# tgm-team/tgm

Hardware: AMD Instinct MI355X
Metric: sampled-edges/sec (TGAT 2-hop k=20 recency sampler, tgbl-wiki synthetic) (higher is better)
Workload: dtype int32/int64 indices + f32 feature rows (copied, no arithmetic)

## Files before the change

### include/tgm_amd.h

```cpp
#ifndef TGM_AMD_H
#define TGM_AMD_H

#include <stddef.h>
#include <stdint.h>

#ifdef __cplusplus
extern "C" {
#endif

#define TGMX_ABI_VERSION 7

#define TGMX_OK 0
#define TGMX_E_INVALID (-1)
#define TGMX_E_LAUNCH (-2)
#define TGMX_E_UNSUPPORTED (-3)

#define TGMX_ST_SEED_RANGE 1
#define TGMX_ST_SEED_TIME 2
#define TGMX_ST_EDGE_RANGE 4
#define TGMX_ST_SCRATCH 8
#define TGMX_ST_TS_BOUND 16

typedef void* tgmx_stream_t;
typedef void* tgmx_event_t;
// ... 69 lines not shown
  float* out_x[TGMX_MAX_HOPS];
  const int32_t* src;
  const int32_t* dst;
  const int64_t* ts;
  const float* edge_x;
  int64_t n, eid0;
  int32_t directed, key_wrap32;
  int32_t* scratch;
  int32_t* status;
  int32_t timed_hop;
  tgmx_event_t ev_start, ev_stop;
  int64_t ts_bound;
  int32_t neg_group, neg_low, neg_high;
  uint64_t neg_seed, neg_call;
  int32_t* neg_out;
  int64_t* neg_time_out;
  int32_t guard_seed_errors;
  int32_t sorted_ts;
  int32_t* out_valid[TGMX_MAX_HOPS];
  int32_t* out_valid_prev[TGMX_MAX_HOPS];
  int64_t neg_index0;
  int64_t* csr_cursor;
  int32_t csr_x_by_pos;
  int32_t* out_eid[TGMX_MAX_HOPS];
  struct tgmx_defer* defer;
  int32_t defer_ok;
} tgmx_recency_step_t;

int tgmx_recency_step(const tgmx_recency_step_t* step, tgmx_stream_t stream);
#define TGMX_PLAN_FUSED01 1
#define TGMX_RIDE_NONE 0
#define TGMX_RIDE_SORT 1
#define TGMX_RIDE_MERGE 2
#define TGMX_RIDE_SORT_MERGE 3
#define TGMX_RIDE_PLACE_ONLY 4
#define TGMX_RIDE_ALL 5
#define TGMX_RIDE_SORT_MERGE_PLACE 6
#define TGMX_RIDE_MERGE_PLACE 7
#define TGMX_AFTER_NONE 0
#define TGMX_AFTER_COMMIT 1
#define TGMX_AFTER_PRESORTED 2
#define TGMX_AFTER_MERGE_PRESORTED 3
#define TGMX_AFTER_BLOCK 4
#define TGMX_AFTER_LARGE 5
int tgmx_recency_step_plan(const tgmx_recency_step_t* step);

typedef struct tgmx_defer tgmx_defer_t;
tgmx_defer_t* tgmx_defer_create(int32_t num_nodes, int32_t B);
void tgmx_defer_destroy(tgmx_defer_t* d);
int tgmx_defer_pending(const tgmx_defer_t* d);
int64_t tgmx_defer_count(const tgmx_defer_t* d);
int tgmx_defer_flush(tgmx_defer_t* d, tgmx_stream_t stream);
int32_t tgmx_set_fused_rows(int32_t rows);

#define TGMX_SEED_SRC 0
#define TGMX_SEED_DST 1
#define TGMX_SEED_NEG 2
typedef struct tgmx_pipeline {
  const int32_t* src;
  const int32_t* dst;
  const int64_t* ts;
  const float* edge_x;
  int64_t num_edges;
  int32_t rank, world;
  int32_t n_roles;
  int32_t seed_role[TGMX_MAX_SEED_GROUPS];
  int32_t neg_low, neg_high;
  uint64_t neg_seed;
  int32_t update;
  int32_t reserved0;
  tgmx_recency_step_t step;
} tgmx_pipeline_t;

typedef struct tgmx_pipeline_out {
  int32_t* neg;
  int64_t* neg_time;
  int32_t* seed_nid0;
  int64_t* seed_ts0;
  int32_t* out_nid[TGMX_MAX_HOPS];
  int64_t* out_ts[TGMX_MAX_HOPS];
  float* out_x[TGMX_MAX_HOPS];
  int32_t timed_hop;
  tgmx_event_t ev_start, ev_stop;
  int32_t* out_valid[TGMX_MAX_HOPS];
  int32_t* out_valid_prev[TGMX_MAX_HOPS];
  int32_t* out_eid[TGMX_MAX_HOPS];
} tgmx_pipeline_out_t;

typedef struct tgmx_pipeline_post {
  int32_t dedup;
  int32_t dedup_neg, dedup_nbr;
  int32_t num_nodes;
  void* dedup_ws;
  int32_t* uniq_out;
  int32_t edge_hop;
  int64_t edge_cap;
  int64_t* row_off;
  int64_t* edge_index;
  int64_t* edge_t;
  float* edge_x;
  int64_t* dev_sizes;
  int64_t* host_sizes;
  tgmx_event_t sizes_ready;
} tgmx_pipeline_post_t;

typedef void* tgmx_worker_t;
// ... 778 lines not shown
```

### tgm_amd/_native.py

```python
from __future__ import annotations

import ctypes
import os
from ctypes import c_char_p, c_int32, c_int64, c_size_t, c_void_p
from typing import Optional

import torch

from .exceptions import NativeLibraryError

_HERE = os.path.dirname(os.path.abspath(__file__))
LIB_PATH = os.path.join(_HERE, 'csrc', 'libtgm_amd.so')

_P = c_void_p
SIGNATURES = {
    'tgmx_version': (c_int32, []),
    'tgmx_abi_sizeof': (c_size_t, [c_int32]),
    'tgmx_last_error': (c_char_p, []),
    'tgmx_event_create': (c_int32, [ctypes.POINTER(c_void_p)]),
    'tgmx_event_destroy': (c_int32, [_P]),
    'tgmx_event_elapsed_ms': (c_int32, [_P, _P, ctypes.POINTER(ctypes.c_float)]),
    'tgmx_recency_lookup_csr': (
        c_int32,
        [_P, _P, _P, c_int32, _P, _P, c_int64, c_int32, c_int32, c_int64, c_int64, c_int32, c_int32, _P, _P, _P, _P, _P, _P, _P],
# ... 243 lines not shown
        ('table', c_void_p), ('ch', c_void_p * 4), ('ldch', c_int64 * 4),
        ('x', c_void_p), ('y', c_void_p), ('x1', c_void_p), ('att', c_void_p), ('qkv', c_void_p), ('h', c_void_p), ('mean', c_void_p),
        ('ldx', c_int64), ('ldq', c_int64), ('ldh', c_int64),
        ('out', c_void_p),
    ]


class TconvFwd(ctypes.Structure):

    _fields_ = [
        ('x', c_void_p), ('U', c_int64), ('in_ch', c_int32), ('last_update_local', c_void_p),
        ('src', c_void_p), ('tgt', c_void_p), ('t', c_void_p), ('msg', c_void_p), ('E', c_int64), ('D', c_int32), ('T', c_int32),
        ('tw', c_void_p), ('tb', c_void_p), ('W4', c_void_p), ('b4', c_void_p), ('W_edge', c_void_p), ('H', c_int32), ('C', c_int32),
        ('edge_attr', c_void_p), ('qkvs', c_void_p), ('eproj', c_void_p), ('order', c_void_p), ('seg_lo', c_void_p), ('seg_hi', c_void_p),
        ('sort_ws', c_void_p), ('sort_ws_bytes', c_size_t), ('status', c_void_p),
        ('tgt_count', c_void_p), ('cursor', c_void_p), ('order_big', c_void_p),
    ]


SEED_SRC, SEED_DST, SEED_NEG = 0, 1, 2


class Pipeline(ctypes.Structure):

    _fields_ = [
        ('src', c_void_p), ('dst', c_void_p), ('ts', c_void_p), ('edge_x', c_void_p), ('num_edges', c_int64),
        ('rank', c_int32), ('world', c_int32), ('n_roles', c_int32), ('seed_role', c_int32 * MAX_SEED_GROUPS),
        ('neg_low', c_int32), ('neg_high', c_int32), ('neg_seed', ctypes.c_uint64),
        ('update', c_int32), ('reserved0', c_int32), ('step', RecencyStep),
    ]


class PipelineOut(ctypes.Structure):

    _fields_ = [
        ('neg', c_void_p), ('neg_time', c_void_p), ('seed_nid0', c_void_p), ('seed_ts0', c_void_p),
        ('out_nid', c_void_p * MAX_HOPS), ('out_ts', c_void_p * MAX_HOPS), ('out_x', c_void_p * MAX_HOPS),
        ('timed_hop', c_int32), ('ev_start', c_void_p), ('ev_stop', c_void_p),
        ('out_valid', c_void_p * MAX_HOPS), ('out_valid_prev', c_void_p * MAX_HOPS), ('out_eid', c_void_p * MAX_HOPS),
    ]


ACCOUNTING_PARTIALS = 1024
SIGNATURES['tgmx_lookup_accounting'] = (c_int32, [_P, c_int64, _P, _P, c_int64, _P, _P])
SIGNATURES['tgmx_uniform_lookup_csr'] = (c_int32, [_P, _P, _P, c_int32, _P, c_int64, c_int32, c_int64, c_int32, c_int32, ctypes.c_uint64, ctypes.c_uint64,
                                                   _P, _P, _P, _P, _P])
SIGNATURES['tgmx_ring_update_scratch_bytes'] = (c_size_t, [c_int64, c_int32])
SIGNATURES['tgmx_defer_create'] = (c_void_p, [c_int32, c_int32])
SIGNATURES['tgmx_defer_destroy'] = (None, [_P])
SIGNATURES['tgmx_defer_pending'] = (c_int32, [_P])
SIGNATURES['tgmx_defer_count'] = (c_int64, [_P])
SIGNATURES['tgmx_defer_flush'] = (c_int32, [_P, _P])
SIGNATURES['tgmx_set_fused_rows'] = (c_int32, [c_int32])
SIGNATURES['tgmx_tgn_gru_gate_backward'] = (c_int32, [_P, _P, _P, _P, c_int32, c_int64, _P, _P, _P])
SIGNATURES['tgmx_tgn_aggregate_backward'] = (c_int32, [c_int64, _P, _P, _P, _P, _P, _P, c_int32, c_int32, _P, _P, c_int32, c_int32, _P, _P, _P])
SIGNATURES['tgmx_tconv_edge_attr_backward'] = (c_int32, [_P, _P, _P, _P, _P, _P, c_int32, c_int32, c_int64, _P, _P])
SIGNATURES['tgmx_tconv_attend_backward'] = (c_int32, [_P, _P, _P, _P, _P, _P, _P, _P, c_int64, c_int32, c_int32, ctypes.c_float, _P, _P, _P, _P, _P, _P, _P])
SIGNATURES['tgmx_group_ids'] = (c_int32, [_P, c_int32, _P, _P, _P, _P, _P, _P])
SIGNATURES['tgmx_group_ids_workspace_bytes'] = (c_size_t, [c_int64])
SIGNATURES['tgmx_group_ids_large'] = (c_int32, [_P, c_int64, _P, _P, _P, _P, _P, _P, c_size_t, _P])
SIGNATURES['tgmx_random_negatives'] = (c_int32, [c_int32, c_int32, c_int64, ctypes.c_uint64, ctypes.c_uint64, _P, _P, c_int64, _P, _P])
SIGNATURES['tgmx_random_negatives_at'] = (c_int32, [c_int32, c_int32, c_int64, ctypes.c_uint64, ctypes.c_uint64, c_int64, _P, _P, c_int64, _P, _P])
SIGNATURES['tgmx_unique_ids_workspace_bytes'] = (c_size_t, [c_int32])
SIGNATURES['tgmx_unique_ids'] = (c_int32, [_P, _P, c_int32, c_int32, _P, _P, _P, _P, _P])
SIGNATURES['tgmx_csr_build_workspace_bytes'] = (c_size_t, [c_int64, c_int32, c_int32])
SIGNATURES['tgmx_csr_build'] = (c_int32, [_P, _P, _P, c_int64, c_int32, _P, c_int64, c_int32, _P, _P, _P, c_size_t, _P, _P])
SIGNATURES['tgmx_recency_step'] = (c_int32, [ctypes.POINTER(RecencyStep), _P])
SIGNATURES['tgmx_recency_step_plan'] = (c_int32, [ctypes.POINTER(RecencyStep)])
SIGNATURES['tgmx_pipeline_step'] = (c_int32, [ctypes.POINTER(Pipeline), c_int64, c_int64, ctypes.c_uint64, ctypes.POINTER(PipelineOut), ctypes.POINTER(PipelinePost), _P])
SIGNATURES['tgmx_event_synchronize'] = (c_int32, [_P])
SIGNATURES['tgmx_event_create_sync'] = (c_int32, [ctypes.POINTER(c_void_p)])
SIGNATURES['tgmx_event_record'] = (c_int32, [_P, _P])
SIGNATURES['tgmx_stream_wait_event'] = (c_int32, [_P, _P])
SIGNATURES['tgmx_stream_handoff'] = (c_int32, [_P, _P, _P])
SIGNATURES['tgmx_worker_create'] = (c_int32, [ctypes.POINTER(c_void_p)])
SIGNATURES['tgmx_worker_destroy'] = (c_int32, [_P])
SIGNATURES['tgmx_worker_pipeline_step'] = (c_int32, [_P, ctypes.POINTER(Pipeline), c_int64, c_int64, ctypes.c_uint64, ctypes.POINTER(PipelineOut),
                                                     ctypes.POINTER(PipelinePost), _P, _P, _P, ctypes.POINTER(ctypes.c_uint64)])
SIGNATURES['tgmx_worker_wait'] = (c_int32, [_P, ctypes.c_uint64])
SIGNATURES['tgmx_slice'] = (c_int32, [_P, c_int64, c_int32, c_int64, c_int32, c_int64, c_int64, c_int64, ctypes.POINTER(c_int64), ctypes.POINTER(c_int64)])
SIGNATURES['tgmx_discretize_workspace_bytes'] = (c_size_t, [c_int64])
SIGNATURES['tgmx_discretize_keep'] = (c_int32, [_P, _P, _P, c_int64, ctypes.c_double, _P, _P, _P, _P, c_size_t, _P])
SIGNATURES['tgmx_tgn_memory_forward'] = (c_int32, [ctypes.POINTER(TgnMemoryFwd), _P])
SIGNATURES['tgmx_tconv_forward'] = (c_int32, [ctypes.POINTER(TconvFwd), _P])
SIGNATURES['tgmx_tgn_step'] = (c_int32, [ctypes.POINTER(TgnStep), _P])
SIGNATURES['tgmx_segment_sort_workspace_bytes'] = (c_size_t, [c_int64])
SIGNATURES['tgmx_segment_sort'] = (c_int32, [_P, c_int64, c_int32, _P, _P, _P, _P, c_size_t, _P, _P])
SIGNATURES['tgmx_tgat_tile16_floats'] = (c_size_t, [c_int32, c_int32])
SIGNATURES['tgmx_tgat_tile16'] = (c_int32, [_P, c_int64, c_int32, c_int32, _P, _P])
SIGNATURES['tgmx_pack2d'] = (c_int32, [ctypes.POINTER(PackJob), c_int32, _P])

SIGNATURES['tgmx_pair_dedup_workspace_bytes'] = (c_size_t, [c_int64])
SIGNATURES['tgmx_pair_dedup'] = (c_int32, [_P, _P, c_int64, _P, _P, _P, _P, _P, c_size_t, _P])
SIGNATURES['tgmx_tgat_layout'] = (c_int32, [ctypes.POINTER(TgatModel), c_int64, ctypes.POINTER(TgatHop), c_int32, ctypes.POINTER(TgatLayout)])
SIGNATURES['tgmx_tgat_workspace_bytes'] = (c_size_t, [ctypes.POINTER(TgatModel), c_int64, ctypes.POINTER(TgatHop)])
SIGNATURES['tgmx_tgat_backward_workspace_bytes'] = (c_size_t, [ctypes.POINTER(TgatModel), ctypes.POINTER(TgatLayout), ctypes.POINTER(TgatHop)])
SIGNATURES['tgmx_tgat_backward'] = (c_int32, [ctypes.POINTER(TgatModel), ctypes.POINTER(TgatLayout), ctypes.POINTER(TgatHop), _P, _P, c_int64,
                                              ctypes.POINTER(Dropout), ctypes.POINTER(TgatGrads), _P, c_size_t, _P])
SIGNATURES['tgmx_tgat_forward'] = (
    c_int32,
    [ctypes.POINTER(TgatModel), _P, c_int64, _P, c_int64, ctypes.POINTER(TgatHop), _P, c_size_t, c_int32, _P, _P],
)

SIGNATURES['tgmx_sgemm_nt_ep'] = (c_int32, [_P, c_int64, _P, c_int64, _P, c_int64, c_int64, c_int32, c_int32, _P, c_int32, _P, c_int64, _P])
SIGNATURES['tgmx_time_gap_workspace_bytes'] = (c_size_t, [c_int64])
SIGNATURES['tgmx_time_gap_group'] = (c_int32, [_P, _P, c_int64, c_int64, _P, c_int64, _P, c_int64, _P, c_int64, _P, c_size_t, _P, _P, _P, _P])
# ... 420 lines not shown
```

### tgm_amd/csrc/recency.hip

```cpp
#include <algorithm>
#include <atomic>
#include <cstdlib>
#include <cstring>
#include <string>
#include <vector>

#include <hip/hip_ext.h>
#include <rocprim/block/block_radix_sort.hpp>
#include <rocprim/block/block_scan.hpp>
#include <rocprim/device/device_radix_sort.hpp>
#include <rocprim/device/device_scan.hpp>
#include <rocprim/iterator/counting_iterator.hpp>
#include <rocprim/iterator/transform_iterator.hpp>

#include "common.h"

namespace tgmx {

struct __align__(16) Rec {
  int nbr;
  int eid;
  long long ts;
};
static_assert(sizeof(Rec) == sizeof(tgmx_adj_t), "record layout");

struct SeedGroups {
  const int32_t* nid[TGMX_MAX_SEED_GROUPS];
  const int64_t* ts[TGMX_MAX_SEED_GROUPS];
  long long end[TGMX_MAX_SEED_GROUPS];
  int32_t* out_nid;
  int64_t* out_ts;
  int groups;
  int gen;
  int gen_low;
  unsigned gen_range;
  unsigned long long gen_seed, gen_call, gen_index0;
  int32_t* gen_out;
  int64_t* gen_out_ts;
};

struct LookupArgs {
  SeedGroups grp;
  const int64_t* indptr;
  const Rec* recs;
  const int32_t* write_pos;
  const float* edge_x;
  const int32_t* seeds;
  const int64_t* qtimes;
  int32_t* out_nid;
  int64_t* out_ts;
  float* out_x;
  int32_t* status;
  long long S;
  long long ev_lo, ev_hi;
  int D, k, B, N, allow_pad;
  int row_vecs;
  FastDiv dv;
  FastDiv dv_seed;
  int32_t* out_eid;
  int32_t* out_eid1;
  int x_by_pos;
  long long* cursor;
  int leave_room;
  unsigned side_blocks;
  int side_stage;
  unsigned commit_blocks;
  const unsigned long long* phdr;
  const Rec* prec;
  const int32_t* pslot;
  const float* pstore;
  unsigned pstamp;
  int peid0;
  int k1;
  int32_t* out_nid1;
  int64_t* out_ts1;
  float* out_x1;
  int32_t* out_valid;
  int32_t* out_valid1;
  int32_t* out_valid_prev;
  int32_t* out_valid_prev1;
  int fused_rows;
  long long* ts;
};

template <int VEC>
struct VecOf;
template <>
struct VecOf<4> { using type = float4; };
template <>
struct VecOf<2> { using type = float2; };
template <>
struct VecOf<1> { using type = float; };

template <typename T>
__device__ __forceinline__ T zero_vec();
template <>
__device__ __forceinline__ float4 zero_vec<float4>() { return make_float4(0.f, 0.f, 0.f, 0.f); }
template <>
__device__ __forceinline__ float2 zero_vec<float2>() { return make_float2(0.f, 0.f); }
template <>
__device__ __forceinline__ float zero_vec<float>() { return 0.f; }

__device__ __forceinline__ long long wave_prefix_count(const Rec* recs, long long a, long long z,
                                                       long long bound, int lane) {
  long long lo = a, hi = z;
  while (hi - lo > kWave) {
    const long long len = hi - lo;
    const long long stride = (len + kWave - 1) / kWave;
    long long idx = lo + (long long)(lane + 1) * stride - 1;
    if (idx > hi - 1) idx = hi - 1;
    const bool less = (long long)recs[idx].eid < bound;
    const int c = __popcll(__ballot(less));
    long long nlo = lo, nhi = hi;
    if (c > 0) {
      long long p = lo + (long long)c * stride - 1;
      if (p > hi - 1) p = hi - 1;
      nlo = p + 1;
    }
    if (c < kWave) {
      long long p = lo + (long long)(c + 1) * stride - 1;
      if (p > hi - 1) p = hi - 1;
      nhi = p;
    }
    lo = nlo;
    hi = nhi < nlo ? nlo : nhi;
  }
  const long long idx = lo + lane;
  const bool less = idx < hi && (long long)recs[idx].eid < bound;
  return lo + __popcll(__ballot(less)) - a;
}

struct UpdateArgs {
  Rec* ring;
  int32_t* write_pos;
// ... 1045 lines not shown
  r.ts = __shfl(r.ts, from_slot);
  src = __shfl(src, from_slot);
  if (a.out_eid || a.out_eid1) r.eid = __shfl(r.eid, from_slot);
  return pick_select<true>(a, w, r, src, q, k, lane);
}

template <bool RING>
__device__ __forceinline__ SmallPick small_pick(const LookupArgs& a, int n, long long q, int k, bool live, int lane) {
  if constexpr (RING) {
    return pick_finish(a, pick_issue(a, n, live, lane), n, q, k, live, lane);
  } else {
    const Window w = find_window<RING>(a, n, live, lane);
    Rec r;
    r.nbr = -1; r.eid = 0; r.ts = 0;
    if (lane < w.wlen) r = a.recs[slot_of<RING>(w, a.B, lane)];
    return pick_select<RING>(a, w, r, -1, q, k, lane);
  }
}

template <int VEC>
__device__ __forceinline__ void gather_rows(const LookupArgs& a, long long s, int k, int lane, const int* lds_eid, float* out_x, int first_slot) {
  using V = typename VecOf<VEC>::type;
  const V* __restrict__ X = reinterpret_cast<const V*>(a.edge_x);
  const int lim = a.pstore ? a.N * a.B : 0x7fffffff;
  const V* __restrict__ P = a.pstore ? reinterpret_cast<const V*>(a.pstore) : X;
  V* __restrict__ O = reinterpret_cast<V*>(out_x + s * (long long)k * a.D);
  const int total = k * a.row_vecs;
  constexpr int U = 8;
  for (int f0 = first_slot * a.row_vecs + lane; f0 < total; f0 += kWave * U) {
    const V* ptr[U];
    bool has[U];
#pragma unroll
    for (int u = 0; u < U; ++u) {
      const int f = f0 + u * kWave;
      const int fc = f < total ? f : f0;
      const int slot = (int)a.dv.div_nb((uint32_t)fc);
      const int col = fc - slot * a.row_vecs;
      const int e = lds_eid[slot];
      has[u] = e >= 0;
      const bool st = e >= lim;
      ptr[u] = (st ? P : X) + (has[u] ? (long long)(st ? e - lim : e) * a.row_vecs + col : 0);
    }
    V v[U];
#pragma unroll
    for (int u = 0; u < U; ++u) v[u] = *ptr[u];
#pragma unroll
    for (int u = 0; u < U; ++u) {
      const int f = f0 + u * kWave;
      if (f < total) O[f] = has[u] ? v[u] : zero_vec<V>();
    }
  }
}

template <bool RING, int VEC, bool SMALL>
__device__ __forceinline__ void lookup_seed(const LookupArgs& a, long long s, int n, long long q, int k, int lane, int* lds_eid,
                                            int32_t* out_nid, int64_t* out_ts, float* out_x, int32_t* out_valid, int32_t* out_valid_prev,
                                            int32_t* out_eid = nullptr) {
  const bool live = n >= 0 && n < a.N;
  int v_new = 0;
  if (SMALL) {
    const SmallPick o = small_pick<RING>(a, n, q, k, live, lane);
    if (lane < k) {
      out_nid[s * k + lane] = o.nbr;
      out_ts[s * k + lane] = o.ts;
      if (out_eid) out_eid[s * k + lane] = o.eid;
      lds_eid[lane] = o.src;
    }
    const unsigned long long m = __ballot(lane < k && o.has);
    v_new = m ? k - __builtin_ctzll(m) : 0;
  } else {
    const int B = a.B;
    const Window w = find_window<RING>(a, n, live, lane);
    int cnt = 0;
    for (int top = w.wlen; top > 0 && cnt == 0; top -= kWave) {
      const int lo = top > kWave ? top - kWave : 0;
      const int i = lo + lane;
      bool ok = false;
      if (i < top) {
        const Rec r = a.recs[slot_of<RING>(w, B, i)];
        ok = r.nbr >= 0 && r.ts < q;
      }
      const unsigned long long m = __ballot(ok);
      if (m) cnt = lo + 64 - __clzll((long long)m);
    }
    for (int c = lane; c < k; c += kWave) {
      const int i = cnt - k + c;
      Rec r;
      r.nbr = -1; r.eid = 0; r.ts = 0;
      if (i >= 0) r = a.recs[slot_of<RING>(w, B, i)];
      const bool has = r.nbr >= 0;
      out_nid[s * k + c] = has ? r.nbr : -1;
      out_ts[s * k + c] = has ? r.ts : 0;
      if (out_eid) out_eid[s * k + c] = has ? r.eid : -1;
      lds_eid[c] = has ? ((RING || a.x_by_pos) ? (int)slot_of<RING>(w, B, i) : r.eid) : -1;
      if (has && k - c > v_new) v_new = k - c;
    }
    for (int o = 32; o > 0; o >>= 1) {
      const int other = __shfl_xor(v_new, o);
      v_new = other > v_new ? other : v_new;
    }
  }
  if (a.D == 0 || out_x == nullptr) return;
  int first_slot = 0;
  if (out_valid) {
    const int v_old = out_valid[s];
    first_slot = k - (v_old > v_new ? v_old : v_new);
    if (lane == 0) {
      out_valid[s] = v_new;
      if (out_valid_prev) out_valid_prev[s] = v_old;
    }
  }
  __builtin_amdgcn_wave_barrier();
  gather_rows<VEC>(a, s, k, lane, lds_eid, out_x, first_slot);
  __builtin_amdgcn_wave_barrier();
}

template <bool RING, int VEC, bool SMALL, bool RIDE>
__global__ __launch_bounds__(256) void recency_lookup_kernel(const LookupArgs a, const UpdateArgs u) {
  extern __shared__ __attribute__((aligned(16))) int lds_eid_all[];
  unsigned bid = blockIdx.x, nblk = gridDim.x;
  if constexpr (RING && RIDE) {
    if (bid < a.side_blocks) {
      update_side_work(u, a.side_stage, (int)bid);
      return;
    }
    bid -= a.side_blocks;
    nblk -= a.side_blocks;
  }
  const int lane = lane_id();
  const int wave_in_block = threadIdx.x >> 6;
  int* lds_eid = lds_eid_all + wave_in_block * a.k;
  const long long waves_total = (long long)nblk * (blockDim.x >> 6);
  for (long long s = (long long)bid * (blockDim.x >> 6) + wave_in_block; s < a.S; s += waves_total) {
    int n;
    long long q;
    fetch_seed(a, s, lane, true, n, q);
    check_seed(a, n, q, a.allow_pad, lane);
    lookup_seed<RING, VEC, SMALL>(a, s, n, q, a.k, lane, lds_eid, a.out_nid, a.out_ts, a.out_x, a.out_valid, a.out_valid_prev, a.out_eid);
  }
}

constexpr int kFusedTsWords = 8;
constexpr int kFusedRowsDefault = 0;
enum FusedTsRole : long long { kTsRider = 1, kTsCommit = 2, kTsHop0 = 3, kTsHop1 = 4 };
__device__ __forceinline__ long long ts_after(int v) {
  asm volatile("" ::"v"(v));
  return (long long)wall_clock64();
}

template <bool RING>
__device__ __forceinline__ SmallPick fused_row_pick(const LookupArgs& a, const PickLoads& L, int n, long long q, bool live, int lane) {
  if constexpr (RING) return pick_finish(a, L, n, q, a.k1, live, lane);
  else return small_pick<false>(a, n, q, a.k1, live, lane);
}

template <bool RING, int VEC, int PCAP = kRidePlaceMaxM, bool ROWS = false, bool TS = false>
__global__ __launch_bounds__(256) void recency_lookup_fused01_kernel(const LookupArgs a, const UpdateArgs u, const UpdateArgs c) {
  extern __shared__ __attribute__((aligned(16))) int lds_eid_all[];
  unsigned bid = blockIdx.x, nblk = gridDim.x;
  const int lane = lane_id();
  const int wave_in_block = threadIdx.x >> 6;
  long long* ts_rec = TS ? a.ts + ((long long)blockIdx.x * (blockDim.x >> 6) + wave_in_block) * kFusedTsWords : nullptr;
  const long long t_start = TS ? (long long)wall_clock64() : 0;
  if constexpr (RING) {
    if (bid < a.side_blocks) {
      update_side_work<PCAP>(u, a.side_stage, (int)bid);
      if (TS && lane == 0) {
        ts_rec[0] = t_start;
        ts_rec[1] = (long long)wall_clock64();
        ts_rec[2] = kTsRider;
      }
      return;
    }
    bid -= a.side_blocks;
    if (bid < a.commit_blocks) {
      commit_block(c, bid);
      if (TS && lane == 0) {
        ts_rec[0] = t_start;
        ts_rec[1] = (long long)wall_clock64();
        ts_rec[2] = kTsCommit;
      }
      return;
    }
    bid -= a.commit_blocks;
    nblk -= a.side_blocks + a.commit_blocks;
  }
  const int k0 = a.k, k1 = a.k1;
  int* lds_eid = lds_eid_all + wave_in_block * (k0 > k1 ? k0 : k1);
  const long long waves_total = (long long)nblk * (blockDim.x >> 6);
  const long long S0 = a.S;
  const int G = ROWS ? a.fused_rows : 0;
  const int runs = G > 0 ? (k0 + G - 1) / G : k0;
  long long role = 0, t_seed = 0, t_index = 0, t_gather = 0;
  for (long long w = (long long)bid * (blockDim.x >> 6) + wave_in_block; w < S0 + S0 * runs; w += waves_total) {
    int n;
    long long q;
    if (w < S0) {
      role = kTsHop0;
      fetch_seed(a, w, lane, true, n, q);
      check_seed(a, n, q, 0, lane);
      lookup_seed<RING, VEC, true>(a, w, n, q, k0, lane, lds_eid, a.out_nid, a.out_ts, a.out_x, a.out_valid, a.out_valid_prev, a.out_eid);
    } else if (!ROWS) {
      role = kTsHop1;
      const long long idx = w - S0;
      const long long s0 = idx / k0;
      const int j = (int)(idx - s0 * k0);
      int n0;
      long long q0;
      fetch_seed(a, s0, lane, false, n0, q0);
      const SmallPick o = small_pick<RING>(a, n0, q0, k0, n0 >= 0 && n0 < a.N, lane);
      n = __shfl(o.nbr, j);
      q = __shfl(o.ts, j);
      lookup_seed<RING, VEC, true>(a, idx, n, q, k1, lane, lds_eid, a.out_nid1, a.out_ts1, a.out_x1, a.out_valid1, a.out_valid_prev1, a.out_eid1);
    } else {
      const long long run = w - S0;
      const long long s0 = run / runs;
      const int j0 = (int)(run - s0 * runs) * G;
      const int rows = k0 - j0 < G ? k0 - j0 : G;
      const long long base = s0 * k0 + j0;
      const bool feats = a.D > 0 && a.out_x1 != nullptr;
      const int v_old_run = (feats && a.out_valid1 && lane < rows) ? a.out_valid1[base + lane] : 0;
      int n0;
      long long q0;
      fetch_seed(a, s0, lane, false, n0, q0);
      const SmallPick o0 = small_pick<RING>(a, n0, q0, k0, n0 >= 0 && n0 < a.N, lane);
      n = __shfl(o0.nbr, j0);
      q = __shfl(o0.ts, j0);
      bool live = n >= 0 && n < a.N;
      if (TS) {
        role = kTsHop1 | ((long long)rows << 8);
        t_seed = ts_after(n);
      }
      PickLoads L = RING ? pick_issue(a, n, live, lane) : PickLoads{};
      for (int r = 0; r < rows; ++r) {
        const long long s = base + r;
        const long long t0 = TS ? (long long)wall_clock64() : 0;
        const SmallPick o = fused_row_pick<RING>(a, L, n, q, live, lane);
        if (lane < k1) {
          a.out_nid1[s * k1 + lane] = o.nbr;
          a.out_ts1[s * k1 + lane] = o.ts;
          if (a.out_eid1) a.out_eid1[s * k1 + lane] = o.eid;
          lds_eid[lane] = o.src;
        }
        const unsigned long long m = __ballot(lane < k1 && o.has);
        const int v_new = m ? k1 - __builtin_ctzll(m) : 0;
        if (TS) {
          const long long t1 = ts_after(v_new);
          t_index += t1 - t0;
        }
        if (r + 1 < rows) {
          n = __shfl(o0.nbr, j0 + r + 1);
          q = __shfl(o0.ts, j0 + r + 1);
          live = n >= 0 && n < a.N;
          if (RING) L = pick_issue(a, n, live, lane);
        }
        if (!feats) continue;
        int first_slot = 0;
        if (a.out_valid1) {
          const int v_old = __shfl(v_old_run, r);
          first_slot = k1 - (v_old > v_new ? v_old : v_new);
          if (lane == 0) {
            a.out_valid1[s] = v_new;
            if (a.out_valid_prev1) a.out_valid_prev1[s] = v_old;
          }
        }
        const long long t2 = TS ? (long long)wall_clock64() : 0;
        __builtin_amdgcn_wave_barrier();
        gather_rows<VEC>(a, s, k1, lane, lds_eid, a.out_x1, first_slot);
        __builtin_amdgcn_wave_barrier();
        if (TS) t_gather += (long long)wall_clock64() - t2;
      }
    }
  }
  if (TS && lane == 0) {
    ts_rec[0] = t_start;
    ts_rec[1] = (long long)wall_clock64();
    ts_rec[2] = role;
    ts_rec[3] = t_seed;
    ts_rec[4] = t_index;
    ts_rec[5] = t_gather;
  }
}

struct GroupPick {
  bool has;
  int nbr, src;
  long long ts;
};

template <bool RING, int GL>
__device__ __forceinline__ GroupPick group_pick(const LookupArgs& a, int n, long long q, int k, bool live, int gl, int sub) {
  const int B = a.B;
  long long w0 = 0;
  int wrot = 0, wlen = 0;
  if constexpr (RING) {
    w0 = (long long)(live ? n : 0) * B;
    wrot = live ? a.write_pos[n] % B : 0;
    wlen = live ? B : 0;
  } else {
    const long long ra = live ? a.indptr[n] : 0, rz = live ? a.indptr[n + 1] : 0;
    const long long p_hi = ra + group_prefix_count<GL>(a.recs, ra, rz, a.ev_hi, gl, sub);
    const long long p_lo = a.ev_lo <= 0 ? ra : ra + group_prefix_count<GL>(a.recs, ra, rz, a.ev_lo, gl, sub);
    w0 = p_hi - B > p_lo ? p_hi - B : p_lo;
    wlen = (int)(p_hi - w0);
  }
  Rec r;
  r.nbr = -1; r.eid = 0; r.ts = 0;
  if (gl < wlen) r = a.recs[w0 + gl];
  if constexpr (RING) {
    int from_slot = wrot + gl;
    if (from_slot >= B) from_slot -= B;
    if (gl >= B) from_slot = gl;
    r.nbr = __shfl(r.nbr, sub * GL + from_slot);
    r.ts = __shfl(r.ts, sub * GL + from_slot);
  }
  const bool ok = gl < wlen && r.nbr >= 0 && r.ts < q;
  const unsigned long long m = (__ballot(ok) >> (sub * GL)) & ((GL == 64) ? ~0ull : ((1ull << GL) - 1));
  const int cnt = m ? 64 - __clzll((long long)m) : 0;
  const int i = cnt - k + gl;
  const int from = i > 0 ? i : 0;
  const int g_nbr = __shfl(r.nbr, sub * GL + from);
  const int g_eid = __shfl(r.eid, sub * GL + from);
  const long long g_ts = __shfl(r.ts, sub * GL + from);
  GroupPick o;
  o.has = i >= 0 && g_nbr >= 0;
  o.nbr = o.has ? g_nbr : -1;
  o.ts = o.has ? g_ts : 0;
  int sl = wrot + from;
  if (sl >= B) sl -= B;
  o.src = o.has ? ((RING || a.x_by_pos) ? (int)(w0 + sl) : g_eid) : -1;
  return o;
}

// ... 722 lines not shown
    if (vec == 4) TGMX_LAUNCH(4, true);
    else if (vec == 2) TGMX_LAUNCH(2, true);
    else TGMX_LAUNCH(1, true);
  } else {
    if (vec == 4) TGMX_LAUNCH(4, false);
    else if (vec == 2) TGMX_LAUNCH(2, false);
    else TGMX_LAUNCH(1, false);
  }
#undef TGMX_LAUNCH
  TGMX_CHECK_LAUNCH("recency_lookup");
  return TGMX_OK;
}


static const char* fused_ts_path() {
  static const char* p = getenv("TGMX_FUSED_TS");
  return (p && *p) ? p : nullptr;
}

static int fused_ts_dump(const LookupArgs& a, hipStream_t stream, unsigned blocks_total, unsigned waves_per_block) {
  static unsigned long long launches = 0;
  const long long waves = (long long)blocks_total * waves_per_block;
  std::vector<long long> h((size_t)(8 + waves * kFusedTsWords));
  if (hipStreamSynchronize(stream) != hipSuccess ||
      hipMemcpy(h.data() + 8, a.ts, (size_t)waves * kFusedTsWords * sizeof(long long), hipMemcpyDeviceToHost) != hipSuccess) {
    set_error("recency_lookup_fused01: reading the timestamps failed");
    return TGMX_E_LAUNCH;
  }
  int dev = 0, khz = 0;
  (void)hipGetDevice(&dev);
  (void)hipDeviceGetAttribute(&khz, hipDeviceAttributeWallClockRate, dev);
  const long long hdr[8] = {0x54474d5854530001ll, waves, (long long)a.side_blocks, (long long)a.commit_blocks, a.S, a.k, a.fused_rows, khz};
  std::copy(hdr, hdr + 8, h.begin());
  const std::string path = std::string(fused_ts_path()) + "." + std::to_string(launches++ % 16);
  if (FILE* f = fopen(path.c_str(), "wb")) {
    fwrite(h.data(), sizeof(long long), h.size(), f);
    fclose(f);
  }
  return TGMX_OK;
}

static std::atomic<int> g_fused_rows{-1};

static int fused_rows_per_wave(int k0) {
  int g = g_fused_rows.load(std::memory_order_relaxed);
  if (g < 0) {
    const char* e = getenv("TGMX_FUSED_ROWS");
    g = (e && *e && atoi(e) >= 0) ? atoi(e) : kFusedRowsDefault;
    g_fused_rows.store(g, std::memory_order_relaxed);
  }
  return g > k0 ? k0 : g;
}

template <bool RING>
static int launch_fused01(LookupArgs a, hipStream_t stream, hipEvent_t ev_start, hipEvent_t ev_stop, const UpdateArgs* side,
                          int side_stage, unsigned side_blocks, int pcap, const UpdateArgs* commit = nullptr) {
  const UpdateArgs u = side ? *side : UpdateArgs{};
  const UpdateArgs c = (RING && commit) ? *commit : UpdateArgs{};
  a.side_blocks = (RING && side) ? side_blocks : 0;
  a.side_stage = side_stage;
  a.commit_blocks = (RING && commit) ? (unsigned)((c.m + 3) / 4) : 0u;
  a.fused_rows = fused_rows_per_wave(a.k);
  const int kmax = a.k > a.k1 ? a.k : a.k1;
  const int vec = prepare_lookup(a, a.out_x1, kmax);
  if (vec < 0) return vec;
  const int waves_per_block = 4;
  const long long runs = a.fused_rows > 0 ? (a.k + a.fused_rows - 1) / a.fused_rows : a.k;
  const long long waves = a.S + a.S * runs;
  long long blocks = (waves + waves_per_block - 1) / waves_per_block;
  if (blocks > (1 << 20)) blocks = 1 << 20;
  const dim3 grid((unsigned)blocks + a.side_blocks + a.commit_blocks), block(waves_per_block * kWave);
  const size_t lds = (size_t)waves_per_block * kmax * sizeof(int);
  if (!(RING && side)) pcap = kRidePlaceMaxM;
  if (RING && vec == 4 && pcap == 512 && fused_ts_path()) {
    static long long* ts_buf = nullptr;
    static size_t ts_cap = 0;
    const size_t need = (size_t)grid.x * waves_per_block * kFusedTsWords * sizeof(long long);
    if (need > ts_cap) {
      if (ts_buf) (void)hipFree(ts_buf);
      ts_buf = nullptr;
      if (hipMalloc(&ts_buf, need) != hipSuccess) {
        set_error("recency_lookup_fused01: no memory for the timestamps");
        return TGMX_E_LAUNCH;
      }
      ts_cap = need;
    }
    a.ts = ts_buf;
    (void)hipMemsetAsync(a.ts, 0, need, stream);
    if (a.fused_rows > 0) TGMX_LAUNCH_TIMED((recency_lookup_fused01_kernel<true, 4, 512, true, true>), grid, block, lds, stream, ev_start, ev_stop, a, u, c);
    else TGMX_LAUNCH_TIMED((recency_lookup_fused01_kernel<true, 4, 512, false, true>), grid, block, lds, stream, ev_start, ev_stop, a, u, c);
    TGMX_CHECK_LAUNCH("recency_lookup_fused01");
    return fused_ts_dump(a, stream, grid.x, waves_per_block);
  }
#define TGMX_FUSED(ROWS_)                                                                                                                            \
  do {                                                                                                                                               \
    if (vec == 4 && pcap == 512) TGMX_LAUNCH_TIMED((recency_lookup_fused01_kernel<RING, 4, RING ? 512 : 1024, ROWS_>), grid, block, lds, stream, ev_start, ev_stop, a, u, c); \
    else if (vec == 4 && pcap == 0) TGMX_LAUNCH_TIMED((recency_lookup_fused01_kernel<RING, 4, RING ? 0 : 1024, ROWS_>), grid, block, lds, stream, ev_start, ev_stop, a, u, c); \
    else if (vec == 4) TGMX_LAUNCH_TIMED((recency_lookup_fused01_kernel<RING, 4, kRidePlaceMaxM, ROWS_>), grid, block, lds, stream, ev_start, ev_stop, a, u, c);            \
    else if (vec == 2) TGMX_LAUNCH_TIMED((recency_lookup_fused01_kernel<RING, 2, kRidePlaceMaxM, ROWS_>), grid, block, lds, stream, ev_start, ev_stop, a, u, c);            \
    else TGMX_LAUNCH_TIMED((recency_lookup_fused01_kernel<RING, 1, kRidePlaceMaxM, ROWS_>), grid, block, lds, stream, ev_start, ev_stop, a, u, c);                          \
  } while (0)
  if (a.fused_rows > 0) TGMX_FUSED(true);
  else TGMX_FUSED(false);
#undef TGMX_FUSED
  TGMX_CHECK_LAUNCH("recency_lookup_fused01");
  return TGMX_OK;
}


__global__ __launch_bounds__(256) void ring_update_span_kernel(const UpdateArgs a) {
  __shared__ long long red[256 / kWave];
  const long long per = (a.n + gridDim.x - 1) / gridDim.x;
  const long long lo = (long long)blockIdx.x * per, hi = lo + per < a.n ? lo + per : a.n;
  long long mx = -0x7fffffffffffffffLL;
  if (lo < hi) mx = strided_max_ts(a.ts + lo, hi - lo, threadIdx.x, 256);
  for (int off = 32; off > 0; off >>= 1) {
    const long long o = __shfl_xor(mx, off);
    mx = o > mx ? o : mx;
  }
// ... 681 lines not shown
  bool pending;
  long long deferred;
  UpdateArgs pend;
};

extern "C" tgmx_defer_t* tgmx_defer_create(int32_t num_nodes, int32_t B) {
  if (num_nodes <= 0 || B <= 0) {
    set_error("defer_create: bad arguments");
    return nullptr;
  }
  auto* d = new tgmx_defer{};
  d->N = num_nodes;
  d->B = B;
  return d;
}

extern "C" void tgmx_defer_destroy(tgmx_defer_t* d) {
  if (d && d->mem) (void)hipFree(d->mem);
  delete d;
}

static int defer_buffers(tgmx_defer* d, hipStream_t st) {
  if (d->mem) return TGMX_OK;
  auto up = [](size_t x) { return (x + 255) & ~(size_t)255; };
  const size_t nb = (size_t)d->N * d->B;
  const size_t half = up(tgmx_ring_update_scratch_bytes(kRidePlaceMaxM, 1));
  const size_t o_scr = up((size_t)16 * d->N), o_slot = o_scr + 2 * half, o_rec = up(o_slot + 8 * nb), total = o_rec + 32 * nb;
  void* mem = nullptr;
  if (hipMalloc(&mem, total) != hipSuccess) {
    set_error("recency_step: cannot allocate %zu bytes for the deferred commit", total);
    return TGMX_E_LAUNCH;
  }
  (void)hipMemsetAsync(mem, 0, o_rec, st);
  char* base = static_cast<char*>(mem);
  d->mem = mem;
  for (int q = 0; q < 2; ++q) {
    d->hdr[q] = reinterpret_cast<unsigned long long*>(base) + (size_t)q * d->N;
    d->scratch[q] = reinterpret_cast<int32_t*>(base + o_scr + q * half);
    d->slot[q] = reinterpret_cast<int32_t*>(base + o_slot) + q * nb;
    d->rec[q] = reinterpret_cast<Rec*>(base + o_rec) + q * nb;
  }
  return TGMX_OK;
}

extern "C" int tgmx_defer_pending(const tgmx_defer_t* d) { return d && d->pending ? 1 : 0; }

extern "C" int64_t tgmx_defer_count(const tgmx_defer_t* d) { return d ? d->deferred : 0; }
extern "C" int32_t tgmx_set_fused_rows(int32_t rows) {
  const int old = fused_rows_per_wave(1 << 30);
  g_fused_rows.store(rows < 0 ? -1 : rows, std::memory_order_relaxed);
  return old;
}

extern "C" int tgmx_defer_flush(tgmx_defer_t* d, tgmx_stream_t stream) {
  TGMX_REQUIRE(d, "defer_flush: null state");
  if (!d->pending) return TGMX_OK;
  d->pending = false;
  hipLaunchKernelGGL(ring_update_feat_kernel<true>, dim3((unsigned)((d->pend.m + 3) / 4)), dim3(256), 0, (hipStream_t)stream, d->pend);
  TGMX_CHECK_LAUNCH("defer_flush");
  return TGMX_OK;
}

static bool getenv_no_ride() {
  static const bool no_ride = getenv("TGMX_NO_RIDE") != nullptr;
  return no_ride;
}


static bool plan_fuse01(const tgmx_recency_step_t* s, long long S0) {
  static const bool no_fuse = getenv("TGMX_NO_FUSE") != nullptr;
  if (no_fuse || s->n_hops < 2 || S0 <= 0 || s->B > kWave || s->k[0] <= 0 || s->k[1] <= 0) return false;
  if (s->indptr != nullptr && (long long)s->k[1] * s->D * 4 < 4096) return false;
  static const bool fuse_by_id = !(getenv("TGMX_FUSE_BY_ID") && atoi(getenv("TGMX_FUSE_BY_ID")) == 0);
  const bool by_id = s->out_eid[1] != nullptr && s->out_x[1] == nullptr;
  if (s->indptr == nullptr && !(by_id && fuse_by_id)) {
    LookupArgs a{};
    a.B = s->B; a.D = s->D; a.edge_x = s->ring_x; a.out_x = s->out_x[0];
    if (prepare_lookup(a, s->out_x[1], s->k[1]) < 0) return false;
    if (packed_group_lanes(a, s->k[1], true) < 64) return false;
  }
  return true;
}

struct RiderPlan {
  int stage[2];
  unsigned blocks[2];
  int pcap;
  int after;
};

static RiderPlan plan_riders(long long m, int n_hops, long long S, bool fused, bool rings) {
  if (!rings || m <= 0) return {};
  if (m > kBlockMaxM) return {{}, {}, 0, kAfterLarge};
  if (n_hops <= 0 || S <= 0 || getenv_no_ride()) return {{}, {}, 0, kAfterBlock};
  const unsigned chunks = (unsigned)((m + kChunk - 1) / kChunk);
  if (fused) {
    if (m <= 512) return {{kSideAll}, {1}, 512, kAfterCommit};
    if (m <= kRidePlaceMaxM) return {{kSideSortMergePlace}, {chunks}, 1024, kAfterCommit};
    return {{kSideSortMerge}, {chunks}, 0, kAfterPresorted};
  }
  if (n_hops == 1) return {{kSideSort}, {chunks}, 0, kAfterMergePresorted};
  if (chunks == 1) return {{kSideSortMerge, kSidePlaceOnly}, {1, 1}, 0, kAfterCommit};
  if (m <= kRidePlaceMaxM) return {{kSideSort, kSideMergePlace}, {chunks, chunks}, 0, kAfterCommit};
  return {{kSideSort, kSideMerge}, {chunks, chunks}, 0, kAfterPresorted};
}

// ... 203 lines not shown
```

Baseline: 9.654 billion.

## Reorder fused hop-1 row-to-wave mapping and prefetch valid counts

Changes how hop-1 waves in the fused two-hop lookup kernel map to (seed, neighbour) rows. A permuted order interleaves seed groups (src/dst/neg) and visits neighbour slots in reverse quads, so concurrently running waves touch a different mix of seeds and adjacency rows. Fast division replaces the 64-bit divide. The old valid count is loaded before the seed fetch so its latency overlaps other loads. It adds a host helper and a setter to choose or inspect the order, plus a timestamp debug field. This risks poorer locality if the permutation spreads accesses.

```diff
diff --git a/include/tgm_amd.h b/include/tgm_amd.h
--- a/include/tgm_amd.h
+++ b/include/tgm_amd.h
@@ -145,6 +145,8 @@
 int64_t tgmx_defer_count(const tgmx_defer_t* d);
 int tgmx_defer_flush(tgmx_defer_t* d, tgmx_stream_t stream);
 int32_t tgmx_set_fused_rows(int32_t rows);
+int32_t tgmx_set_fused_order(int32_t mode);
+int32_t tgmx_fused_row_order(int64_t S0, int32_t k0, int32_t groups, const int64_t* group_end, int32_t mode, int64_t* out_idx);
 
 #define TGMX_SEED_SRC 0
 #define TGMX_SEED_DST 1
diff --git a/tgm_amd/_native.py b/tgm_amd/_native.py
--- a/tgm_amd/_native.py
+++ b/tgm_amd/_native.py
@@ -319,6 +319,8 @@
 SIGNATURES['tgmx_defer_count'] = (c_int64, [_P])
 SIGNATURES['tgmx_defer_flush'] = (c_int32, [_P, _P])
 SIGNATURES['tgmx_set_fused_rows'] = (c_int32, [c_int32])
+SIGNATURES['tgmx_set_fused_order'] = (c_int32, [c_int32])
+SIGNATURES['tgmx_fused_row_order'] = (c_int32, [c_int64, c_int32, c_int32, _P, c_int32, _P])
 SIGNATURES['tgmx_tgn_gru_gate_backward'] = (c_int32, [_P, _P, _P, _P, c_int32, c_int64, _P, _P, _P])
 SIGNATURES['tgmx_tgn_aggregate_backward'] = (c_int32, [c_int64, _P, _P, _P, _P, _P, _P, c_int32, c_int32, _P, _P, c_int32, c_int32, _P, _P, _P])
 SIGNATURES['tgmx_tconv_edge_attr_backward'] = (c_int32, [_P, _P, _P, _P, _P, _P, c_int32, c_int32, c_int64, _P, _P])
diff --git a/tgm_amd/csrc/recency.hip b/tgm_amd/csrc/recency.hip
--- a/tgm_amd/csrc/recency.hip
+++ b/tgm_amd/csrc/recency.hip
@@ -38,6 +38,73 @@
   int32_t* gen_out;
   int64_t* gen_out_ts;
 };
+
+__host__ __device__ __forceinline__ uint32_t fastdiv_of(const FastDiv& f, uint32_t n) {
+  return (uint32_t)(((unsigned long long)n * f.m) >> 32) + (n & f.pass);
+}
+__host__ __device__ __forceinline__ unsigned long long mulhi_u64(unsigned long long x, unsigned long long y) {
+#if defined(__HIP_DEVICE_COMPILE__)
+  return __umul64hi(x, y);
+#else
+  return (unsigned long long)(((unsigned __int128)x * y) >> 64);
+#endif
+}
+
+constexpr int kFusedWaves = 4;
+struct FusedOrder {
+  FastDiv dk0, dS0, dG;
+  uint32_t n;
+  int quads, deal;
+  int wide;
+  unsigned long long m64;
+};
+
+static FusedOrder fused_order_make(long long S0, int k0, int groups, const long long* group_end, int mode) {
+  FusedOrder o{};
+  const long long rows = S0 * k0, big = S0 > k0 ? S0 : k0;
+  o.m64 = k0 >= 2 ? ~0ull / (unsigned long long)k0 + 1ull : 0ull;
+  o.wide = rows <= 0 || big >= (1ll << 32) || rows >= ((1ll << 32) + big - 1) / big;
+  if (o.wide) return o;
+  o.dk0 = make_fastdiv((uint32_t)k0);
+  if (mode >= 1 && groups >= 2 && S0 % groups == 0 && rows * groups < (1ll << 32)) {
+    const long long n = S0 / groups;
+    bool equal = true;
+    for (int g = 0; g < groups; ++g) equal = equal && group_end[g] == (g + 1) * n;
+    if (equal) {
+      o.deal = 1;
+      o.n = (uint32_t)n;
+      o.dG = make_fastdiv((uint32_t)groups);
+    }
+  }
+  if (mode == 2 && k0 % kFusedWaves == 0) {
+    o.quads = 1;
+    o.dS0 = make_fastdiv((uint32_t)S0);
+  }
+  return o;
+}
+
+__host__ __device__ __forceinline__ void fused_row_of(const FusedOrder& o, long long i, int k0, long long S0, long long& s0, int& j) {
+  if (o.wide) {
+    s0 = k0 >= 2 ? (long long)mulhi_u64((unsigned long long)i, o.m64) : i;
+    j = (int)(i - s0 * k0);
+    return;
+  }
+  uint32_t t;
+  if (o.quads) {
+    const uint32_t u = (uint32_t)i / kFusedWaves, r = (uint32_t)i % kFusedWaves;
+    const uint32_t cq = fastdiv_of(o.dS0, u);
+    t = u - cq * (uint32_t)S0;
+    j = (int)(((uint32_t)k0 / kFusedWaves - 1 - cq) * kFusedWaves + r);
+  } else {
+    t = fastdiv_of(o.dk0, (uint32_t)i);
+    j = (int)((uint32_t)i - t * (uint32_t)k0);
+  }
+  if (o.deal) {
+    const uint32_t b = fastdiv_of(o.dG, t);
+    t = (t - b * o.dG.d) * o.n + b;
+  }
+  s0 = t;
+}
 
 struct LookupArgs {
   SeedGroups grp;
@@ -80,6 +147,7 @@
   int32_t* out_valid_prev;
   int32_t* out_valid_prev1;
   int fused_rows;
+  FusedOrder ord;
   long long* ts;
 };
 
@@ -1231,10 +1299,10 @@
   }
 }
 
-template <bool RING, int VEC, bool SMALL>
+template <bool RING, int VEC, bool SMALL, bool PRE = false>
 __device__ __forceinline__ void lookup_seed(const LookupArgs& a, long long s, int n, long long q, int k, int lane, int* lds_eid,
                                             int32_t* out_nid, int64_t* out_ts, float* out_x, int32_t* out_valid, int32_t* out_valid_prev,
-                                            int32_t* out_eid = nullptr) {
+                                            int32_t* out_eid = nullptr, int v_old_pre = 0) {
   const bool live = n >= 0 && n < a.N;
   int v_new = 0;
   if (SMALL) {
@@ -1282,7 +1350,7 @@
   if (a.D == 0 || out_x == nullptr) return;
   int first_slot = 0;
   if (out_valid) {
-    const int v_old = out_valid[s];
+    const int v_old = PRE ? v_old_pre : out_valid[s];
     first_slot = k - (v_old > v_new ? v_old : v_new);
     if (lane == 0) {
       out_valid[s] = v_new;
@@ -1370,27 +1438,37 @@
   const long long S0 = a.S;
   const int G = ROWS ? a.fused_rows : 0;
   const int runs = G > 0 ? (k0 + G - 1) / G : k0;
-  long long role = 0, t_seed = 0, t_index = 0, t_gather = 0;
+  long long role = 0, t_seed = 0, t_index = 0, t_gather = 0, ts_row = -1;
   for (long long w = (long long)bid * (blockDim.x >> 6) + wave_in_block; w < S0 + S0 * runs; w += waves_total) {
     int n;
     long long q;
     if (w < S0) {
       role = kTsHop0;
-      fetch_seed(a, w, lane, true, n, q);
-      check_seed(a, n, q, 0, lane);
-      lookup_seed<RING, VEC, true>(a, w, n, q, k0, lane, lds_eid, a.out_nid, a.out_ts, a.out_x, a.out_valid, a.out_valid_prev, a.out_eid);
+      if constexpr (ROWS) {
+        fetch_seed(a, w, lane, true, n, q);
+        check_seed(a, n, q, 0, lane);
+        lookup_seed<RING, VEC, true>(a, w, n, q, k0, lane, lds_eid, a.out_nid, a.out_ts, a.out_x, a.out_valid, a.out_valid_prev, a.out_eid);
+      } else {
+        const int v_old = (a.D > 0 && a.out_x && a.out_valid) ? a.out_valid[w] : 0;
+        fetch_seed(a, w, lane, true, n, q);
+        check_seed(a, n, q, 0, lane);
+        lookup_seed<RING, VEC, true, true>(a, w, n, q, k0, lane, lds_eid, a.out_nid, a.out_ts, a.out_x, a.out_valid, a.out_valid_prev, a.out_eid, v_old);
+      }
     } else if (!ROWS) {
       role = kTsHop1;
-      const long long idx = w - S0;
-      const long long s0 = idx / k0;
-      const int j = (int)(idx - s0 * k0);
+      long long s0;
+      int j;
+      fused_row_of(a.ord, w - S0, k0, S0, s0, j);
+      const long long idx = s0 * k0 + j;
+      const int v_old = (a.D > 0 && a.out_x1 && a.out_valid1) ? a.out_valid1[idx] : 0;
+      if (TS) ts_row = idx;
       int n0;
       long long q0;
       fetch_seed(a, s0, lane, false, n0, q0);
       const SmallPick o = small_pick<RING>(a, n0, q0, k0, n0 >= 0 && n0 < a.N, lane);
       n = __shfl(o.nbr, j);
       q = __shfl(o.ts, j);
-      lookup_seed<RING, VEC, true>(a, idx, n, q, k1, lane, lds_eid, a.out_nid1, a.out_ts1, a.out_x1, a.out_valid1, a.out_valid_prev1, a.out_eid1);
+      lookup_seed<RING, VEC, true, true>(a, idx, n, q, k1, lane, lds_eid, a.out_nid1, a.out_ts1, a.out_x1, a.out_valid1, a.out_valid_prev1, a.out_eid1, v_old);
     } else {
       const long long run = w - S0;
       const long long s0 = run / runs;
@@ -1458,6 +1536,7 @@
     ts_rec[3] = t_seed;
     ts_rec[4] = t_index;
     ts_rec[5] = t_gather;
+    ts_rec[6] = ts_row;
   }
 }
 
@@ -2286,6 +2365,19 @@
   return g > k0 ? k0 : g;
 }
 
+constexpr int kFusedOrderDefault = 2;
+static std::atomic<int> g_fused_order{-1};
+
+static int fused_order_mode() {
+  int m = g_fused_order.load(std::memory_order_relaxed);
+  if (m < 0) {
+    const char* e = getenv("TGMX_FUSED_ORDER");
+    m = (e && *e && atoi(e) >= 0 && atoi(e) <= 2) ? atoi(e) : kFusedOrderDefault;
+    g_fused_order.store(m, std::memory_order_relaxed);
+  }
+  return m;
+}
+
 template <bool RING>
 static int launch_fused01(LookupArgs a, hipStream_t stream, hipEvent_t ev_start, hipEvent_t ev_stop, const UpdateArgs* side,
                           int side_stage, unsigned side_blocks, int pcap, const UpdateArgs* commit = nullptr) {
@@ -2295,10 +2387,11 @@
   a.side_stage = side_stage;
   a.commit_blocks = (RING && commit) ? (unsigned)((c.m + 3) / 4) : 0u;
   a.fused_rows = fused_rows_per_wave(a.k);
+  a.ord = fused_order_make(a.S, a.k, a.grp.groups, a.grp.end, a.fused_rows > 0 ? 0 : fused_order_mode());
   const int kmax = a.k > a.k1 ? a.k : a.k1;
   const int vec = prepare_lookup(a, a.out_x1, kmax);
   if (vec < 0) return vec;
-  const int waves_per_block = 4;
+  const int waves_per_block = kFusedWaves;
   const long long runs = a.fused_rows > 0 ? (a.k + a.fused_rows - 1) / a.fused_rows : a.k;
   const long long waves = a.S + a.S * runs;
   long long blocks = (waves + waves_per_block - 1) / waves_per_block;
@@ -3086,6 +3179,28 @@
   return old;
 }
 
+extern "C" int32_t tgmx_set_fused_order(int32_t mode) {
+  const int old = fused_order_mode();
+  g_fused_order.store((mode < 0 || mode > 2) ? -1 : mode, std::memory_order_relaxed);
+  return old;
+}
+
+extern "C" int32_t tgmx_fused_row_order(int64_t S0, int32_t k0, int32_t groups, const int64_t* group_end, int32_t mode, int64_t* out_idx) {
+  TGMX_REQUIRE(S0 >= 0 && k0 > 0 && out_idx, "fused_row_order: bad sizes or no output");
+  TGMX_REQUIRE(mode >= 0 && mode <= 2, "fused_row_order: mode is 0, 1 or 2");
+  TGMX_REQUIRE(groups >= 0 && groups <= TGMX_MAX_SEED_GROUPS && (groups == 0 || group_end), "fused_row_order: bad seed groups");
+  long long end[TGMX_MAX_SEED_GROUPS] = {};
+  for (int g = 0; g < groups; ++g) end[g] = group_end[g];
+  const FusedOrder o = fused_order_make(S0, k0, groups, end, mode);
+  for (long long i = 0; i < S0 * k0; ++i) {
+    long long s0;
+    int j;
+    fused_row_of(o, i, k0, S0, s0, j);
+    out_idx[i] = s0 * k0 + j;
+  }
+  return TGMX_OK;
+}
+
 extern "C" int tgmx_defer_flush(tgmx_defer_t* d, tgmx_stream_t stream) {
   TGMX_REQUIRE(d, "defer_flush: null state");
   if (!d->pending) return TGMX_OK;
```

New measurement: 9.864 billion (median of 6 runs). 1.02x the previous value.
